# HuttleyLab/DiverseSeq

Measured on NVIDIA B200. Metric: prep_nmost_throughput, higher is better.
Workload: dtype u8 bases -> u32 counts -> f64 frequencies/entropy/JSD

## Files before the change

diverseseq_b200/csrc/select.cu:

```cuda
#include <limits.h>
#include <stddef.h>
#include <stdlib.h>
#include <string.h>

#include <algorithm>
#include <limits>

#include <cooperative_groups.h>

#include "comm.cuh"
#include "common.cuh"
#include "entropy.cuh"
#include "fused.cuh"

namespace cg = cooperative_groups;

namespace dvs {

constexpr unsigned kNone = 0xFFFFFFFFu;

struct SelScal {
    double E;
    double total_jsd;
    double mean, stdv, cov;
// ... 523 lines not shown
                cudaOccupancyMaxActiveBlocksPerMultiprocessor(&per_sm2, k_sel_persist_sm_full, kFastThreads,
                                                              sizeof(SmShared)) == cudaSuccess &&
                per_sm2 > 0;
        (void)cudaGetLastError();
    }
    const unsigned sm_grid = std::min(std::min<unsigned>((unsigned)ctx->sm_count, kSmMaxGrid), grid_cap);
    const int slim_threads = 128 * (trail_shape() + 1);
    const auto k_slim = slim_threads == 384 ? SlimKernel<384>::fn : (slim_threads == 256 ? SlimKernel<256>::fn : SlimKernel<128>::fn);
    bool slim_ok = false;
    if (trail && sm_ok) {
        slim_ok = cudaFuncSetAttribute(k_slim, cudaFuncAttributeMaxDynamicSharedMemorySize,
                                       (int)sizeof(SmSharedSlim)) == cudaSuccess &&
                  cudaFuncSetAttribute(k_slim, cudaFuncAttributePreferredSharedMemoryCarveout,
                                       (int)cudaSharedmemCarveoutMaxShared) == cudaSuccess;
        (void)cudaGetLastError();
    }
    DevBuf<SlicePart> d_slparts;
    DevBuf<unsigned> d_slticks;
    DevBuf<SmPart> d_spart, d_upart, d_dpart;
    if (sm_ok) {
        DVS_TRY(d_spart.alloc(2 * kSmMaxGrid));
        DVS_TRY(d_upart.alloc(kSmMaxN + 1));
        DVS_TRY(d_dpart.alloc(3));
    }
    const char* gb_env = getenv("DVS_SELECT_GROW_BATCH");
    const bool use_grow_batch = use_fast && grow_mode && !(gb_env && gb_env[0] == '0');
    const unsigned kGrowWindowMax = 64 * world;
    SelState fresh;
    DevBuf<FastSum> d_gparts;
    DevBuf<double> d_gmd, d_gmb;
    DevBuf<SelScal> d_gscratch;
    DevBuf<unsigned> d_ginteresting;
    bool fresh_valid = false;
    unsigned grow_window = 16;
    if (use_grow_batch && n != max_size) {
        DVS_TRY(fresh.alloc(dim, cap));
        DVS_TRY(d_gparts.alloc((size_t)kGrowWindowMax * (cap + 3)));
        DVS_TRY(d_gmd.alloc((size_t)kGrowWindowMax * cap));
        DVS_TRY(d_gmb.alloc((size_t)kGrowWindowMax * cap));
        DVS_TRY(d_gscratch.alloc(kGrowWindowMax));
        DVS_TRY(d_ginteresting.alloc(1));
    }
    unsigned fresh_n = 0;
    const SelState* fresh_of = nullptr;
    int fresh_which = -1;
    bool single_candidate = false;
    unsigned filter_streak = 0, filter_bypass = 0;
    while (cursor < num) {
        if (use_grow_batch && n != max_size && !single_candidate && filter_bypass > 0) {
            --filter_bypass;
            single_candidate = true;
            continue;
        }
        if (use_grow_batch && n != max_size && !single_candidate) {
            if (!fresh_valid || fresh_n != n || fresh_of != cur || fresh_which != cur->which) {
                k_sel_sum<<<sel.vec_grid(), 256, 0, st>>>(f->freqs.p, f->entropy.p, dim, cur->members(), n, -1, fresh.S(),
                                                          fresh.members(), fresh.sc.p);
                DVS_LAUNCHED(ctx);
                fresh_valid = true;
                fresh_n = n;
                fresh_of = cur;
                fresh_which = cur->which;
            }
            const unsigned W = std::min(grow_window, num - cursor);
            DVS_CUDA_TRY(cudaMemsetAsync(d_ginteresting.p, 0xFF, sizeof(unsigned), st));
            const unsigned gc0 = (rank + world - cursor % world) % world;
            const unsigned Wloc = W > gc0 ? (W - gc0 + world - 1) / world : 0;
            if (Wloc) {
                k_grow_eval<<<dim3(n + 3, Wloc), kFastThreads, 0, st>>>(f->freqs.p, dim, cur->S(), cur->members(), cur->sc.p,
                                                                        fresh.S(), f->valid.p, is_member.p, d_order.p,
                                                                        cursor, d_gparts.p, gc0, world);
                DVS_LAUNCHED(ctx);
                k_grow_decide<<<Wloc, kFastThreads, 0, st>>>(f->entropy.p, dim, cur->members(), cur->sc.p, fresh.sc.p,
                                                             f->valid.p, is_member.p, d_order.p, cursor, d_gparts.p, d_gmd.p,
                                                             d_gmb.p, cap, d_gscratch.p, d_ginteresting.p,
                                                             mode == DVS_MODE_MAX_COV ? 1 : 0, gc0, world);
                DVS_LAUNCHED(ctx);
            }
            if (world > 1) DVS_TRY(comm_min_u32(ctx, comm, d_ginteresting.p, d_ginteresting.p));
            unsigned* h_fi = reinterpret_cast<unsigned*>(reinterpret_cast<char*>(ctx->pinned) + sizeof(SelScal));
            DVS_CUDA_TRY(cudaMemcpyAsync(h_fi, d_ginteresting.p, sizeof(unsigned), cudaMemcpyDeviceToHost, st));
            DVS_CUDA_TRY(cudaStreamSynchronize(st));
            const unsigned fi = *h_fi;
            if (fi == kNone) {
                cursor += W;
                grow_window = std::min(grow_window * 2u, kGrowWindowMax);
                continue;
            }
            grow_window = std::max(4u, std::min(kGrowWindowMax, 2u * (fi - cursor + 1u)));
            if (fi == cursor) {
                if (++filter_streak >= 2) filter_bypass = 1u << std::min(filter_streak - 2u, 3u);
            } else {
                filter_streak = 0;
            }
            cursor = fi;
            single_candidate = true;
            continue;
        }
        if (trail && trail_limit < num && !use_persist) {
            DVS_CUDA_TRY(cudaStreamWaitEvent(st, trail->count_done, 0));
            trail_limit = num;
        }
        if (use_persist && (!grow_mode || n == max_size)) {
            const bool use_sm = sm_ok && n <= kSmMaxN;
            const bool dedicated = trail_shape() == 3;
            const bool trailing = trail && trail_limit < num && use_sm && world == 1 &&
                                  (dedicated || (slim_ok && n <= kSmSlimMaxN));
            if (trail && trail_limit < num && !trailing) {
                DVS_CUDA_TRY(cudaStreamWaitEvent(st, trail->count_done, 0));
                trail_limit = num;
            }
            const unsigned grid = (trailing && dedicated) ? std::min(sm_grid, trail_sms(ctx->sm_count))
                                                           : (use_sm ? sm_grid : persist_grid);
            k_sel_set_dev<<<1, 1, 0, st>>>(cur->sc.p, cursor, std::min(window, grid * world), grid * world, num, accepts,
                                           (unsigned)cur->which);
            if (comm) {
                shard.tag_base = (unsigned)((++comm->sel_tag_base) << 20);
                DVS_TRY(comm_host_rendezvous(ctx, comm));
            }
            DVS_LAUNCHED(ctx);
            const double* a_F = f->freqs.p;
            const double* a_H = f->entropy.p;
            uint64_t a_dim = dim;
            double *a_S0 = cur->Sbuf[0].p, *a_S1 = cur->Sbuf[1].p;
            unsigned *a_M0 = cur->membuf[0].p, *a_M1 = cur->membuf[1].p;
            uint8_t* a_mem = is_member.p;
            double *a_md = cur->mdelta.p, *a_mb = cur->mbound.p;
            SelScal* a_sc = cur->sc.p;
            const uint8_t* a_valid = f->valid.p;
            const unsigned* a_order = d_order.p;
            unsigned a_rounds = world > 1 ? 0xFFFF0u : 0x7fffffffu;
            unsigned long long* a_trace = nullptr;
            DevBuf<unsigned long long> d_trace;
            const char* tr_env = getenv("DVS_SELECT_TRACE");
            const char* tra_env = getenv("DVS_SELECT_TRACE_ALL");
            int a_trace_all = (use_sm && tra_env && tra_env[0]) ? 1 : 0;
            const size_t trace_len = a_trace_all ? (size_t)256 * kSmTraceSlots * kSmMaxGrid : 2048;
            if (a_trace_all) tr_env = nullptr;
            if ((tr_env && tr_env[0]) || a_trace_all) {
                DVS_TRY(d_trace.alloc(trace_len));
                DVS_CUDA_TRY(cudaMemsetAsync(d_trace.p, 0, trace_len * sizeof(unsigned long long), st));
                a_trace = d_trace.p;
            }
            if (use_sm) {
                unsigned a_dim32 = (unsigned)dim;
                double* a_S = cur->S();
                unsigned* a_M = cur->members();
                SmPart *a_sp = d_spart.p, *a_up = d_upart.p, *a_dp = d_dpart.p;
                DVS_CUDA_TRY(cudaMemsetAsync(d_dpart.p, 0, 3 * sizeof(SmPart), st));
                DVS_CUDA_TRY(cudaMemsetAsync(d_spart.p, 0, 2 * kSmMaxGrid * sizeof(SmPart), st));
                DVS_CUDA_TRY(cudaMemsetAsync(d_upart.p, 0, (kSmMaxN + 1) * sizeof(SmPart), st));
                const unsigned* a_ready = trailing ? trail->d_ready : nullptr;
                unsigned a_limit0 = trail_limit;
                void* args[] = {&a_F, &a_H, &a_dim32, &a_S, &a_M, &a_mem, &a_md, &a_mb, &a_sc, &a_valid, &a_order,
                                &a_sp, &a_up, &a_dp, &a_trace, &a_trace_all, &shard, &a_ready, &a_limit0};
                if (trailing && dedicated) {
                    if (!ctx->stream_hi) {
                        int lo_p = 0, hi_p = 0;
                        DVS_CUDA_TRY(cudaDeviceGetStreamPriorityRange(&lo_p, &hi_p));
                        DVS_CUDA_TRY(cudaStreamCreateWithPriority(&ctx->stream_hi, cudaStreamNonBlocking, hi_p));
                        DVS_CUDA_TRY(cudaEventCreateWithFlags(&ctx->ev_hi_in, cudaEventDisableTiming));
                        DVS_CUDA_TRY(cudaEventCreateWithFlags(&ctx->ev_hi_out, cudaEventDisableTiming));
                    }
                    DVS_CUDA_TRY(cudaEventRecord(ctx->ev_hi_in, st));
                    DVS_CUDA_TRY(cudaStreamWaitEvent(ctx->stream_hi, ctx->ev_hi_in, 0));
                    k_sel_persist_sm_full<<<grid, kFastThreads, sizeof(SmShared), ctx->stream_hi>>>(
                        a_F, a_H, a_dim32, a_S, a_M, a_mem, a_md, a_mb, a_sc, a_valid, a_order, a_sp, a_up, a_dp, a_trace,
                        a_trace_all, shard, a_ready, a_limit0);
                    DVS_CUDA_TRY(cudaGetLastError());
                    DVS_CUDA_TRY(cudaEventRecord(ctx->ev_hi_out, ctx->stream_hi));
                    DVS_CUDA_TRY(cudaStreamWaitEvent(st, ctx->ev_hi_out, 0));
                } else if (trailing) {
                    k_wait_resident<<<1, 1, 0, st>>>(trail->d_resident, std::min<unsigned>(grid, (unsigned)ctx->sm_count),
                                                     trail->d_ready, num);
                    DVS_LAUNCHED(ctx);
                }
                if (trailing && dedicated) {
                } else if (trailing)
                    k_slim<<<grid, slim_threads, sizeof(SmSharedSlim), st>>>(
                        a_F, a_H, a_dim32, a_S, a_M, a_mem, a_md, a_mb, a_sc, a_valid, a_order, a_sp, a_up, a_dp, a_trace,
                        a_trace_all, shard, a_ready, a_limit0);
                else
                    DVS_CUDA_TRY(cudaLaunchCooperativeKernel((void*)k_sel_persist_sm_full, dim3(grid), dim3(kFastThreads),
                                                             args, sizeof(SmShared), st));
            } else {
                const char* sl_env = getenv("DVS_SELECT_SLICES");
                unsigned a_slice_mode = sl_env ? (unsigned)atoi(sl_env) : 1u;
                if (!d_slparts.p && a_slice_mode) {
                    const size_t slots = std::max<size_t>(grid, (size_t)cap + 1);
                    DVS_TRY(d_slparts.alloc(slots * kMaxSlices));
                    DVS_TRY(d_slticks.alloc(slots));
                    DVS_CUDA_TRY(cudaMemsetAsync(d_slticks.p, 0, slots * sizeof(unsigned), st));
                }
                SlicePart* a_parts = d_slparts.p;
                unsigned* a_ticks = d_slticks.p;
                void* args[] = {&a_F, &a_H, &a_dim, &a_S0, &a_S1, &a_M0, &a_M1, &a_mem, &a_md, &a_mb, &a_sc, &a_valid,
                                &a_order, &a_rounds, &a_trace, &shard, &a_parts, &a_ticks, &a_slice_mode};
                DVS_CUDA_TRY(cudaLaunchCooperativeKernel((void*)k_sel_persist, dim3(grid), dim3(kFastThreads), args, 0, st));
            }
            ctx->launches++;
            DVS_TRY(sel.read(*cur));
            if (a_trace && a_trace_all) {
                std::vector<unsigned long long> tr(trace_len);
                DVS_CUDA_TRY(cudaMemcpy(tr.data(), a_trace, trace_len * sizeof(unsigned long long), cudaMemcpyDeviceToHost));
                if (FILE* fp = fopen(tra_env, "wb")) {
                    fwrite(tr.data(), sizeof(unsigned long long), trace_len, fp);
                    fclose(fp);
                }
            } else if (a_trace) {
                std::vector<unsigned long long> tr(2048);
                DVS_CUDA_TRY(cudaMemcpy(tr.data(), a_trace, 2048 * sizeof(unsigned long long), cudaMemcpyDeviceToHost));
                if (FILE* fp = fopen(tr_env, "a")) {
                    const int slots = use_sm ? kSmTraceSlots : 4, used = use_sm ? 7 : 4;
                    fprintf(fp, use_sm ? "# round scan_ns gather_ns decide_ns update_ns gather2_ns finalize_ns next_ns (CTA 0)\n"
                                       : "# round scan_ns wait1_ns update_ns wait2_ns (CTA 0; wait = grid barrier incl. the slowest CTA)\n");
                    for (int r = 0; (r + 1) * slots < 2048 && tr[slots * (r + 1)]; ++r) {
                        fprintf(fp, "%d", r);
                        for (int q = 0; q + 1 < used; ++q) fprintf(fp, " %llu", tr[slots * r + q + 1] - tr[slots * r + q]);
                        fprintf(fp, " %llu\n", tr[slots * (r + 1)] - tr[slots * r + used - 1]);
                    }
                    fclose(fp);
                }
            }
            const SelScal hd = *sel.h_sc;
            if (hd.panic) return panic_error(hd);
            if (trailing) {
                ctx->last_trail_accepts += hd.accepts - accepts;
                ++ctx->last_trail_launches;
                std::vector<unsigned> smid(grid);
                DVS_CUDA_TRY(cudaMemcpyAsync(smid.data(), trail->d_ready + kTrailSmidOff, grid * sizeof(unsigned),
                                             cudaMemcpyDeviceToHost, st));
                DVS_CUDA_TRY(cudaStreamSynchronize(st));
                std::sort(smid.begin(), smid.end());
                const unsigned distinct = (unsigned)(std::unique(smid.begin(), smid.end()) - smid.begin());
                ctx->last_trail_sms = std::min(ctx->last_trail_sms, distinct);
            }
            cursor = hd.cursor;
            window = hd.window;
            accepts = hd.accepts;
            cur->which = (int)hd.which;
            if (trailing) trail_limit = std::max(trail_limit, std::min(hd.limit, num));
            if (!hd.halt) continue;
            DVS_TRY(sel.reset_scan(*cur));
            if (cursor >= num) break;
        } else if (use_dev && world == 1 && (!grow_mode || n == max_size)) {
            k_sel_set_dev<<<1, 1, 0, st>>>(cur->sc.p, cursor, std::min(window, window_max_dev), window_max_dev, num,
                                           accepts, (unsigned)cur->which);
            DVS_LAUNCHED(ctx);
            for (int r = 0; r < kRoundsPerBatch; ++r) {
                k_sel_scan_dev<<<window_max_dev, kFastThreads, 0, st>>>(
                    f->freqs.p, f->entropy.p, dim, cur->Sbuf[0].p, cur->Sbuf[1].p, cur->membuf[0].p, cur->membuf[1].p,
                    cur->sc.p, f->valid.p, is_member.p, d_order.p);
                DVS_LAUNCHED(ctx);
                k_sel_round_dev<<<n + 1, kFastThreads, 0, st>>>(
                    f->freqs.p, f->entropy.p, dim, cur->Sbuf[0].p, cur->Sbuf[1].p, cur->membuf[0].p, cur->membuf[1].p,
                    is_member.p, cur->mdelta.p, cur->mbound.p, cur->sc.p, d_order.p);
                DVS_LAUNCHED(ctx);
            }
            DVS_TRY(sel.read(*cur));
            const SelScal hd = *sel.h_sc;
            if (hd.panic) return panic_error(hd);
            cursor = hd.cursor;
            window = hd.window;
            accepts = hd.accepts;
            cur->which = (int)hd.which;
            if (!hd.halt) continue;
            DVS_TRY(sel.reset_scan(*cur));
            if (cursor >= num) break;
        }
        if (cursor >= trail_limit) {
            DVS_CUDA_TRY(cudaStreamWaitEvent(st, trail->count_done, 0));
            trail_limit = num;
        }
        const unsigned count = single_candidate ? 1u : std::min(window, trail_limit - cursor);
        single_candidate = false;
        SelScal h;
        unsigned pos = kNone;
        if (use_fast) {
            DVS_TRY(sel.scan_fast(*cur, is_member.p, d_order.p, cursor, count));
            DVS_TRY(sel.read(*cur));
            h = *sel.h_sc;
            if (h.panic) return panic_error(h);
            if (h.state_unsure) {
                DVS_TRY(sel.update(*cur, n));
                ++exact_evals;
                continue;
            }
            if (h.first_unsure < h.first_true) {
                const unsigned pu = h.first_unsure;
                if (!h.exact) DVS_TRY(sel.update(*cur, n));
                DVS_TRY(sel.scan(*cur, f, is_member.p, d_order.p, pu, 1, nullptr));
                DVS_TRY(sel.read(*cur));
                h = *sel.h_sc;
                ++exact_evals;
                if (h.panic) return panic_error(h);
                if (h.first_panic == pu) {
                    set_error("cannot calculate entropy as frequency vector total !=1.0 (candidate at position %u)", pu);
                    return DVS_ERR_VALUE;
                }
                if (h.first_true != pu) {
                    DVS_TRY(sel.reset_scan(*cur));
                    cursor = pu + 1;
                    continue;
                }
                pos = pu;
            } else if (h.first_true != kNone) {
                pos = h.first_true;
            }
        } else {
            DVS_TRY(sel.scan(*cur, f, is_member.p, d_order.p, cursor, count, nullptr));
            DVS_TRY(sel.read(*cur));
            h = *sel.h_sc;
            if (h.panic) return panic_error(h);
            if (h.first_panic != kNone && h.first_panic <= h.first_true) {
                set_error("cannot calculate entropy as frequency vector total !=1.0 (candidate at position %u)",
                          h.first_panic);
                return DVS_ERR_VALUE;
            }
            pos = h.first_true;
        }
        if (pos == kNone) {
            cursor += count;
            window = std::min(window * 2, window_max);
            continue;
        }
        const unsigned row = order[pos];
        window = std::max(64u, std::min(window_max, 2 * (pos - cursor + 1)));
        cursor = pos + 1;
        if (!grow_mode || n == max_size) {
            DVS_TRY(use_fast ? sel.replace_fast(*cur, n, row, is_member.p) : sel.replace(*cur, n, row, is_member.p));
            ++accepts;
            continue;
        }
        const bool use_cov = (mode == DVS_MODE_MAX_COV);
// ... 279 lines not shown
```

diverseseq_b200/csrc/select_fast.cuh:

```cuda
#pragma once

constexpr int kFastThreads = 512;

struct FastSum {
    double e, t, a;
    int bad;
};

template <class Elem>
__device__ FastSum block_entropy_span(uint64_t lo, uint64_t dim, Elem elem) {
    __shared__ double s_part[3][kFastThreads / 32];
    __shared__ int s_bad[kFastThreads / 32];
    double e0 = 0.0, e1 = 0.0, t0 = 0.0, t1 = 0.0, a0 = 0.0, a1 = 0.0;
    int bad = 0;
    constexpr int kBatch = 8;
    for (uint64_t base = lo; base < dim; base += (uint64_t)kBatch * kFastThreads) {
        double x[kBatch];
#pragma unroll
        for (int q = 0; q < kBatch; ++q) {
            const uint64_t i = base + threadIdx.x + (uint64_t)q * kFastThreads;
            x[q] = i < dim ? elem(i) : 0.0;
        }
#pragma unroll
        for (int q = 0; q < kBatch; q += 2) {
            const double x0 = x[q], x1 = x[q + 1];
            if (!(x0 == 0.0)) {
                bad |= !(x0 > 0.0);
                const double tm = __dmul_rn(-x0, log2(x0));
                e0 += tm; a0 += fabs(tm); t0 += x0;
            }
            if (!(x1 == 0.0)) {
                bad |= !(x1 > 0.0);
                const double tm = __dmul_rn(-x1, log2(x1));
                e1 += tm; a1 += fabs(tm); t1 += x1;
            }
        }
    }
    double e = e0 + e1, t = t0 + t1, a = a0 + a1;
    for (int o = 16; o; o >>= 1) {
        e += __shfl_xor_sync(0xffffffffu, e, o);
        t += __shfl_xor_sync(0xffffffffu, t, o);
        a += __shfl_xor_sync(0xffffffffu, a, o);
        bad |= __shfl_xor_sync(0xffffffffu, bad, o);
    }
    const int w = threadIdx.x >> 5;
    if ((threadIdx.x & 31) == 0) {
        s_part[0][w] = e; s_part[1][w] = t; s_part[2][w] = a; s_bad[w] = bad;
    }
    __syncthreads();
    FastSum r{0.0, 0.0, 0.0, 0};
    for (int q = 0; q < kFastThreads / 32; ++q) {
        r.e += s_part[0][q]; r.t += s_part[1][q]; r.a += s_part[2][q]; r.bad |= s_bad[q];
    }
    __syncthreads();
    return r;
}
template <class Elem>
__device__ __forceinline__ FastSum block_entropy_fast(uint64_t dim, Elem elem) {
    return block_entropy_span(0, dim, elem);
}

__device__ __forceinline__ bool fast_term_ok(double m) {
    return (uint32_t)__double2hiint(m) - 0x07b00000u < 0x3feea4afu - 0x07b00000u;
}

template <bool CLAMP, int BATCH, int NT = kFastThreads, class Num>
__device__ FastSum block_entropy_ilp(unsigned lo, unsigned hi, Num num, const FastDiv dv,
                                     const double2* __restrict__ ltab) {
    __shared__ double s_part[3][NT / 32];
    __shared__ int s_bad[NT / 32];
    double e0 = 0.0, e1 = 0.0, t0 = 0.0, t1 = 0.0, a0 = 0.0, a1 = 0.0;
    bool bad = false;
    for (unsigned base = lo; base < hi; base += BATCH * NT) {
        double x[BATCH], l[BATCH];
#pragma unroll
        for (int q = 0; q < BATCH; ++q) {
            const unsigned i = base + threadIdx.x + (unsigned)q * NT;
            x[q] = i < hi ? num(i) : 0.0;
        }
#pragma unroll
        for (int q = 0; q < BATCH; ++q) {
            double m = div_exact(x[q], dv);
            if (CLAMP) m = (m <= kEps) ? 0.0 : m;
            x[q] = m;
        }
#pragma unroll
        for (int q = 0; q < BATCH; ++q) {
            int ignored = 0;
            l[q] = dvs_log2_main(x[q], ltab, ignored);
        }
#pragma unroll
        for (int q = 0; q < BATCH; ++q) {
            const bool ok = fast_term_ok(x[q]);
            bad |= !ok && !(x[q] == 0.0);
            const double tm = ok ? __dmul_rn(-x[q], l[q]) : 0.0;
            if (q & 1) {
                e1 += tm; a1 += fabs(tm); t1 += x[q];
            } else {
                e0 += tm; a0 += fabs(tm); t0 += x[q];
            }
        }
    }
    double e = e0 + e1, t = t0 + t1, a = a0 + a1;
    int badi = bad ? 1 : 0;
    for (int o = 16; o; o >>= 1) {
        e += __shfl_xor_sync(0xffffffffu, e, o);
        t += __shfl_xor_sync(0xffffffffu, t, o);
        a += __shfl_xor_sync(0xffffffffu, a, o);
        badi |= __shfl_xor_sync(0xffffffffu, badi, o);
    }
    const int w = threadIdx.x >> 5;
    if ((threadIdx.x & 31) == 0) {
        s_part[0][w] = e; s_part[1][w] = t; s_part[2][w] = a; s_bad[w] = badi;
    }
    __syncthreads();
    FastSum r{0.0, 0.0, 0.0, 0};
    for (int q = 0; q < NT / 32; ++q) {
        r.e += s_part[0][q]; r.t += s_part[1][q]; r.a += s_part[2][q]; r.bad |= s_bad[q];
    }
    __syncthreads();
    return r;
}

template <bool CLAMP, class Num>
__device__ FastSum block_entropy_div(uint64_t dim, Num num, double divisor) {
    if (dim > (1ull << 30) || !(divisor >= 1.0 && divisor <= 4096.0)) {
        return block_entropy_fast(dim, [&](uint64_t i) {
            const double m = __ddiv_rn(num(i), divisor);
            return (CLAMP && m <= kEps) ? 0.0 : m;
        });
    }
    __shared__ double2 s_ltab_div[64];
    dvs_log2_stage_table(s_ltab_div);
    __syncthreads();
    return block_entropy_ilp<CLAMP, 8>(0u, (unsigned)dim, num, make_fast_div(divisor), s_ltab_div);
}

__device__ __forceinline__ double fast_slack(uint64_t dim, double depth = 0.0) {
    return (double)(dim / kFastThreads) + 12.0 + depth;
}
__device__ __forceinline__ double fast_bound(uint64_t dim, double a, double extra, double depth = 0.0) {
    return ((double)dim + fast_slack(dim, depth) + 16.0) * 1.2e-16 * (a + fabs(extra) + 1.0);
}
__device__ __forceinline__ bool fast_total_ok(uint64_t dim, double t, double depth = 0.0) {
    const double lim = ((double)dim + 1.0 - fast_slack(dim, depth) - 2.0) * 1.1102230246251565e-16;
    return lim > 0.0 && fabs(t - 1.0) <= lim;
}

template <bool GLOBAL = true>
__device__ __forceinline__ unsigned finalize_fast_block(double* mdelta, const double* mbound, unsigned n, double total,
                                                        double total_bound, unsigned* low_out) {
    auto ld = [](const double* p) { return GLOBAL ? __ldcg(p) : *p; };
    __shared__ double s_mn[kFastThreads / 32], s_mb[kFastThreads / 32];
    __shared__ unsigned s_ix[kFastThreads / 32];
    __shared__ double s_best, s_bestb;
    __shared__ unsigned s_besti;
    double mn = 1e300, mb = 0.0;
    unsigned ix = kNone;
    for (unsigned t = threadIdx.x; t < n; t += blockDim.x) {
        const double d = total - ld(&mdelta[t]);
        mdelta[t] = d;
        if (d < mn || (d == mn && t < ix)) {
            mn = d;
            mb = ld(&mbound[t]);
            ix = t;
        }
    }
    for (int o = 16; o; o >>= 1) {
        const double omn = __shfl_xor_sync(0xffffffffu, mn, o), omb = __shfl_xor_sync(0xffffffffu, mb, o);
        const unsigned oix = __shfl_xor_sync(0xffffffffu, ix, o);
        if (omn < mn || (omn == mn && oix < ix)) {
            mn = omn; mb = omb; ix = oix;
        }
    }
    if ((threadIdx.x & 31) == 0) {
        s_mn[threadIdx.x >> 5] = mn; s_mb[threadIdx.x >> 5] = mb; s_ix[threadIdx.x >> 5] = ix;
    }
    __syncthreads();
    if (threadIdx.x == 0) {
        for (unsigned w = 1; w < blockDim.x / 32; ++w)
            if (s_mn[w] < mn || (s_mn[w] == mn && s_ix[w] < ix)) {
                mn = s_mn[w]; mb = s_mb[w]; ix = s_ix[w];
            }
        s_best = mn; s_bestb = mb; s_besti = (ix == kNone) ? 0u : ix;
    }
    __syncthreads();
    mn = s_best; mb = s_bestb;
    const unsigned low = s_besti;
    int unsure = 0;
    for (unsigned t = threadIdx.x; t < n; t += blockDim.x)
        if (t != low && !(mn + mb + 2.0 * kEps < mdelta[t] - ld(&mbound[t]))) unsure = 1;
    if (!(mn + mb + total_bound < 1e6)) unsure = 1;
    unsure = __syncthreads_or(unsure);
    *low_out = low;
    return (unsigned)unsure;
}

__device__ __forceinline__ double block_sum_fast(double v) {
    __shared__ double s_red[kFastThreads / 32];
    __shared__ double s_out;
    for (int o = 16; o; o >>= 1) v += __shfl_xor_sync(0xffffffffu, v, o);
    if ((threadIdx.x & 31) == 0) s_red[threadIdx.x >> 5] = v;
    __syncthreads();
    if (threadIdx.x == 0) {
        double t = 0.0;
        for (unsigned w = 0; w < blockDim.x / 32; ++w) t += s_red[w];
        s_out = t;
    }
    __syncthreads();
    const double r = s_out;
    __syncthreads();
    return r;
}
__device__ __forceinline__ double block_max_fast(double v) {
    __shared__ double s_red[kFastThreads / 32];
    __shared__ double s_out;
    for (int o = 16; o; o >>= 1) v = fmax(v, __shfl_xor_sync(0xffffffffu, v, o));
    if ((threadIdx.x & 31) == 0) s_red[threadIdx.x >> 5] = v;
    __syncthreads();
    if (threadIdx.x == 0) {
        double t = s_red[0];
        for (unsigned w = 1; w < blockDim.x / 32; ++w) t = fmax(t, s_red[w]);
        s_out = t;
    }
    __syncthreads();
    const double r = s_out;
    __syncthreads();
    return r;
}

__device__ __forceinline__ void stats_fast_block(const double* mdelta, const double* mbound, unsigned n,
                                                 double total_bound, SelScal* sc) {
    double sd = 0.0, bmx = 0.0, amx = 0.0;
    for (unsigned t = threadIdx.x; t < n; t += blockDim.x) {
        const double d = mdelta[t];
        sd += d;
        bmx = fmax(bmx, __ldcg(&mbound[t]));
        amx = fmax(amx, fabs(d));
    }
    const double nd = (double)n;
    const double mean = block_sum_fast(sd) / nd;
    bmx = block_max_fast(bmx);
    amx = block_max_fast(amx);
    double ss = 0.0;
    for (unsigned t = threadIdx.x; t < n; t += blockDim.x) {
        const double d = mdelta[t] - mean;
        ss += d * d;
    }
    const double sdev = sqrt(block_sum_fast(ss) / (nd - 1.0));
    if (threadIdx.x == 0) {
        const double u = 1.2e-16, scale = amx + fabs(mean);
        const double b_mean = bmx + total_bound + (nd + 8.0) * u * scale;
        const double b_std = 1.5 * (bmx + 4.0 * u * scale) + (nd + 8.0) * u * sdev;
        const double cov = sdev / mean;
        double b_cov = 1e300;
        if (fabs(mean) > 2.0 * b_mean) b_cov = (b_std + fabs(cov) * b_mean) / (fabs(mean) - b_mean) + 8.0 * u * fabs(cov);
        sc->mean = mean;
        sc->stdv = sdev;
        sc->cov = cov;
        sc->std_bound = b_std;
        sc->cov_bound = b_cov;
    }
}

struct ScanScal {
    double E, total_jsd, total_bound;
    unsigned n, low_row;
};

__device__ __forceinline__ void scan_fast_body(const double* __restrict__ F, const double* __restrict__ H, uint64_t dim,
                                               const double* __restrict__ S, SelScal* sc, const ScanScal& q,
                                               const uint8_t* __restrict__ valid,
                                               const uint8_t* __restrict__ is_member,
                                               const unsigned* __restrict__ order, unsigned pos) {
    const unsigned row = order[pos];
    if (!valid[row] || __ldcg(is_member + row)) return;
    const double nd = (double)q.n;
    const double* fl = F + (size_t)q.low_row * dim;
    const double* fc = F + (size_t)row * dim;
    FastSum h = block_entropy_div<false>(
        dim, [&](uint64_t i) { return __dadd_rn(__dsub_rn(__ldcg(S + i), fl[i]), fc[i]); }, nd);
    if (threadIdx.x == 0) {
        const double mean_entropy = __ddiv_rn(__dadd_rn(__dsub_rn(q.E, H[q.low_row]), H[row]), nd);
        const double d = h.e - mean_entropy;
        const double b = fast_bound(dim, h.a, mean_entropy);
        const double thr = q.total_jsd + kEps, tb = q.total_bound + 4.0 * kEps;
        if (h.bad || !fast_total_ok(dim, h.t) || !(d == d)) {
            atomicMin(&sc->first_unsure, pos);
        } else if (d - b > thr + tb) {
            atomicMin(&sc->first_true, pos);
        } else if (!(d + b < thr - tb)) {
            atomicMin(&sc->first_unsure, pos);
// ... 471 lines not shown
```

diverseseq_b200/csrc/select_sm.cuh:

```cuda
#pragma once

constexpr unsigned kSmMaxDim = 4096, kSmMaxN = 1024, kSmMaxGrid = 256, kSmChunk = 4 * kFastThreads;
constexpr double kSmDepth = 4.0;

struct __align__(16) SmPart {
    unsigned long long w[4];
};

template <unsigned MAXN, unsigned CHUNK>
struct SmSharedT {
    double S[kSmMaxDim];
    double mH[2][MAXN + 1];
    double md[MAXN + 1];
    double mb[MAXN + 1];
    unsigned members[2][MAXN + 1];
    double cH[CHUNK];
    unsigned crow[CHUNK];
    unsigned char cvalid[CHUNK];
    double pe[kSmMaxGrid], pt[kSmMaxGrid], pa[kSmMaxGrid];
    unsigned char pbad[kSmMaxGrid], wskip[kSmMaxGrid];
    unsigned ft, fu, unsure, xft, xfu, dead, limit;
    double2 ltab[64];
};
using SmShared = SmSharedT<kSmMaxN, kSmChunk>;
constexpr unsigned kSmSlimMaxN = 256, kSmSlimChunk = 1280;
using SmSharedSlim = SmSharedT<kSmSlimMaxN, kSmSlimChunk>;

__device__ __forceinline__ void sm_st128(void* p, unsigned long long lo, unsigned long long hi) {
    asm volatile("{ .reg .b128 v; mov.b128 v, {%1, %2}; st.relaxed.gpu.global.b128 [%0], v; }" ::"l"(p), "l"(lo), "l"(hi)
                 : "memory");
}
__device__ __forceinline__ void sm_ld128(const void* p, unsigned long long& lo, unsigned long long& hi) {
    asm volatile("{ .reg .b128 v; ld.relaxed.gpu.global.b128 v, [%2]; mov.b128 {%0, %1}, v; }"
                 : "=l"(lo), "=l"(hi)
                 : "l"(p)
                 : "memory");
}
__device__ __forceinline__ void sm_publish(SmPart* slot, const FastSum& h, unsigned tag) {
    sm_st128(&slot->w[0], (unsigned long long)__double_as_longlong(h.e), ((unsigned long long)(h.bad ? 1u : 0u) << 32) | tag);
    sm_st128(&slot->w[2], (unsigned long long)__double_as_longlong(h.t),
             ((unsigned long long)__float_as_uint(__double2float_ru(h.a)) << 32) | tag);
}
__device__ __forceinline__ FastSum sm_gather(const SmPart* slot, unsigned tag) {
    unsigned long long w0, w1, w2, w3;
    do sm_ld128(&slot->w[0], w0, w1); while ((unsigned)w1 != tag);
    do sm_ld128(&slot->w[2], w2, w3); while ((unsigned)w3 != tag);
    return FastSum{__longlong_as_double((long long)w0), __longlong_as_double((long long)w2),
                   (double)__uint_as_float((unsigned)(w3 >> 32)), (int)(w1 >> 32)};
}

template <int NT>
__device__ __forceinline__ unsigned sm_finalize(double* md, const double* mb_, unsigned n, double total,
                                                double total_bound, unsigned* low_out) {
    __shared__ double s_mn[NT / 32], s_mb[NT / 32];
    __shared__ unsigned s_ix[NT / 32];
    double mn = 1e300, mb = 0.0;
    unsigned ix = kNone;
    for (unsigned t = threadIdx.x; t < n; t += blockDim.x) {
        const double d = total - md[t];
        md[t] = d;
        if (d < mn || (d == mn && t < ix)) {
            mn = d; mb = mb_[t]; ix = t;
        }
    }
    for (int o = 16; o; o >>= 1) {
        const double omn = __shfl_xor_sync(0xffffffffu, mn, o), omb = __shfl_xor_sync(0xffffffffu, mb, o);
        const unsigned oix = __shfl_xor_sync(0xffffffffu, ix, o);
        if (omn < mn || (omn == mn && oix < ix)) {
            mn = omn; mb = omb; ix = oix;
        }
    }
    if ((threadIdx.x & 31) == 0) {
        s_mn[threadIdx.x >> 5] = mn; s_mb[threadIdx.x >> 5] = mb; s_ix[threadIdx.x >> 5] = ix;
    }
    __syncthreads();
    mn = s_mn[0]; mb = s_mb[0]; ix = s_ix[0];
#pragma unroll
    for (unsigned w = 1; w < NT / 32; ++w) {
        const double wmn = s_mn[w];
        const unsigned wix = s_ix[w];
        if (wmn < mn || (wmn == mn && wix < ix)) {
            mn = wmn; mb = s_mb[w]; ix = wix;
        }
    }
    const unsigned low = (ix == kNone) ? 0u : ix;
    int unsure = 0;
    for (unsigned t = threadIdx.x; t < n; t += blockDim.x)
        if (t != low && !(mn + mb + 2.0 * kEps < md[t] - mb_[t])) unsure = 1;
    if (!(mn + mb + total_bound < 1e6)) unsure = 1;
    unsure = __syncthreads_or(unsure);
    *low_out = low;
    return (unsigned)unsure;
}

constexpr int kSmTraceSlots = 8;
constexpr unsigned kTrailSmidOff = 64;

template <int NT, int MINB, unsigned MAXN, unsigned CHUNK>
__global__ void __launch_bounds__(NT, MINB)
k_sel_persist_sm_t(const double* __restrict__ F, const double* __restrict__ H, unsigned dim, double* S_glob,
                 unsigned* M_glob, uint8_t* is_member, double* mdelta_g, double* mbound_g, SelScal* sc,
                 const uint8_t* __restrict__ valid, const unsigned* __restrict__ order, SmPart* spart, SmPart* upart,
                 SmPart* dpart, unsigned long long* trace, int trace_all, const ShardArgs sh,
                 const unsigned* ready_pos, unsigned limit0) {
    extern __shared__ __align__(16) unsigned char sm_raw[];
    SmSharedT<MAXN, CHUNK>& sm = *reinterpret_cast<SmSharedT<MAXN, CHUNK>*>(sm_raw);
    const unsigned tid = threadIdx.x, b = blockIdx.x, G = gridDim.x;
    if (ready_pos && tid == 0) {
        unsigned smid;
        asm volatile("mov.u32 %0, %%smid;" : "=r"(smid));
        const_cast<unsigned*>(ready_pos)[kTrailSmidOff + b] = smid;
    }
    unsigned tr_round = 0;
    auto stamp = [&](int slot) {
        if (trace && tid == 0 && tr_round < 256 && (b == 0 || trace_all)) {
            unsigned long long t;
            asm volatile("mov.u64 %0, %%globaltimer;" : "=l"(t));
            if (trace_all)
                trace[((size_t)tr_round * kSmTraceSlots + slot) * kSmMaxGrid + b] = t;
            else
                trace[tr_round * kSmTraceSlots + slot] = t;
        }
    };

    const unsigned n = sc->n, num = sc->num;
    const double nd = (double)n, div = __dsub_rn(nd, 1.0);
    const FastDiv div_n = make_fast_div(nd), div_n1 = make_fast_div(div);
    double E = sc->E, total_jsd = sc->total_jsd, total_bound = sc->total_bound;
    unsigned lowest = sc->lowest, cursor = sc->cursor, window = sc->window, accepts = sc->accepts;
    unsigned state_unsure = sc->state_unsure, halt = state_unsure ? 1u : 0u, mw = 0;
    bool touched = false;
    dvs_log2_stage_table(sm.ltab);
    for (unsigned i = tid; i < dim; i += NT) sm.S[i] = S_glob[i];
    for (unsigned j = tid; j < n; j += NT) {
        const unsigned r = M_glob[j];
        sm.members[0][j] = r;
        sm.mH[0][j] = H[r];
    }
    __syncthreads();
    const unsigned world = (unsigned)sh.world, rank = (unsigned)sh.rank, Gw = G * world;
    const unsigned wmin = max(1u, Gw / 4u);
    if (tid == 0) sm.dead = 0;
    const double kb0 = ((double)dim + fast_slack(dim) + 16.0) * 1.2e-16;
    const double kb4 = ((double)dim + fast_slack(dim, kSmDepth) + 16.0) * 1.2e-16;
    const double lim0 = ((double)dim + 1.0 - fast_slack(dim) - 2.0) * 1.1102230246251565e-16;
    const double lim4 = ((double)dim + 1.0 - fast_slack(dim, kSmDepth) - 2.0) * 1.1102230246251565e-16;
    auto total_ok = [](double t, double lim) { return lim > 0.0 && fabs(t - 1.0) <= lim; };
    unsigned xs = 0, xu = 0;
    unsigned cbase = 0, cend = 0;
    unsigned limit = ready_pos ? min(limit0, num) : num;

    while (!halt && cursor < num) {
        stamp(0);
        if (xs >= 0xFFFF0u) {
            halt = 1;
            break;
        }
        if (ready_pos && limit >= num) break;
        window = max(1u, min(window, min(Gw, CHUNK)));
        const unsigned P = (dim >= 2048u && window * 4u <= Gw) ? 4u : ((dim >= 2048u && window * 2u <= Gw) ? 2u : 1u);
        const unsigned count = min(window, limit - cursor);
        const unsigned woff = (rank + world - cursor % world) % world;
        const unsigned nloc = count > woff ? (count - woff + world - 1u) / world : 0u;
        if (cursor < cbase || cursor + count > cend) {
            __syncthreads();
            cbase = cursor;
            cend = min(limit, cbase + CHUNK);
            for (unsigned q = tid; cbase + q < cend; q += NT) {
                const unsigned row = order[cbase + q];
                sm.crow[q] = row;
                sm.cvalid[q] = __ldcg(valid + row);
                sm.cH[q] = __ldcg(H + row);
            }
            for (unsigned r = (rank + world - cbase % world) % world + world * b; r < cend - cbase; r += world * G) {
                const double* fr = F + (size_t)order[cbase + r] * dim;
                for (unsigned l = tid * 16u; l < dim; l += NT * 16u)
                    asm volatile("prefetch.global.L2 [%0];" ::"l"(fr + l));
            }
            __syncthreads();
        }
        const unsigned coff = cursor - cbase;
        if (tid == 0) {
            sm.ft = kNone;
            sm.fu = kNone;
        }
        for (unsigned q = tid; q < nloc; q += NT) sm.wskip[q] = sm.cvalid[coff + woff + world * q] ? 0 : 1;
        ++xs;
        SmPart* const sbuf = spart + (xs & 1u) * kSmMaxGrid;
        const unsigned c = b / P, p = b % P;
        const unsigned cw = woff + world * c;
        const double* fl = F + (size_t)sm.members[mw][lowest] * dim;
        if (c < nloc && sm.cvalid[coff + cw]) {
            const double* fc = F + (size_t)sm.crow[coff + cw] * dim;
            const unsigned lo = (unsigned)(((uint64_t)dim * p) / P), hi = (unsigned)(((uint64_t)dim * (p + 1)) / P);
            auto num = [&](unsigned i) { return __dadd_rn(__dsub_rn(sm.S[i], fl[i]), fc[i]); };
            const FastSum h = P == 4u   ? block_entropy_ilp<false, 2, NT>(lo, hi, num, div_n, sm.ltab)
                              : P == 2u ? block_entropy_ilp<false, 4, NT>(lo, hi, num, div_n, sm.ltab)
                                        : block_entropy_ilp<false, 8, NT>(lo, hi, num, div_n, sm.ltab);
            if (tid == 0) sm_publish(sbuf + b, h, xs);
        } else if (tid == 0) {
            sm_publish(sbuf + b, FastSum{0.0, 0.0, 0.0, 0}, xs);
        }
        stamp(1);
        SmPart* const dslot = dpart + (xs & 1u);
        if (b == 0) {
            __syncthreads();
            for (unsigned j = tid; j < n; j += NT) {
                const unsigned r = sm.members[mw][j];
                for (unsigned cc = 0; cc < nloc; ++cc)
                    if (sm.crow[coff + woff + world * cc] == r) sm.wskip[cc] = 1;
            }
            __syncthreads();
            for (unsigned q = tid; q < G; q += NT) {
                const FastSum g = sm_gather(sbuf + q, xs);
                if (q < nloc * P && !sm.wskip[q / P]) {
                    sm.pe[q] = g.e; sm.pt[q] = g.t; sm.pa[q] = g.a; sm.pbad[q] = (unsigned char)g.bad;
                }
            }
            __syncthreads();
            stamp(2);
            for (unsigned lc = tid; lc < nloc; lc += NT) {
                if (sm.wskip[lc]) continue;
                FastSum h{sm.pe[lc * P], sm.pt[lc * P], sm.pa[lc * P], sm.pbad[lc * P]};
                for (unsigned q = 1; q < P; ++q) {
                    h.e += sm.pe[lc * P + q]; h.t += sm.pt[lc * P + q]; h.a += sm.pa[lc * P + q];
                    h.bad |= sm.pbad[lc * P + q];
                }
                const unsigned pos = cursor + woff + world * lc;
                const double mean_entropy =
                    div_exact(__dadd_rn(__dsub_rn(E, sm.mH[mw][lowest]), sm.cH[pos - cbase]), div_n);
                const double d = h.e - mean_entropy;
                const double bd = (P > 1u ? kb4 : kb0) * (h.a + fabs(mean_entropy) + 1.0);
                const double thr = total_jsd + kEps, tb = total_bound + 4.0 * kEps;
                if (h.bad || !total_ok(h.t, P > 1u ? lim4 : lim0) || !(d == d)) {
                    atomicMin(&sm.fu, pos);
                } else if (d - bd > thr + tb) {
                    atomicMin(&sm.ft, pos);
                } else if (!(d + bd < thr - tb)) {
                    atomicMin(&sm.fu, pos);
                }
            }
            __syncthreads();
            if (world > 1u) {
                const unsigned lft = sm.ft, lfu = sm.fu;
                __syncthreads();
                shard_exchange_min(sh, xs, lft, lfu, &sm.ft, &sm.fu, &sm.dead);
                __syncthreads();
                if (sm.dead) {
                    if (tid == 0) {
                        sm.ft = kNone;
                        sm.fu = 0u;
                        sc->panic = 2u;
                    }
                    __syncthreads();
                }
            }
            if (tid == 0) {
                unsigned nl = limit;
                if (ready_pos) nl = max(limit, min(num, *reinterpret_cast<const volatile unsigned*>(ready_pos)));
                sm.limit = nl;
                sm_st128(&dslot->w[0], ((unsigned long long)sm.fu << 32) | sm.ft, ((unsigned long long)nl << 32) | xs);
            }
            __syncthreads();
        } else {
            if (tid == 0) {
                unsigned long long w0, w1;
                do sm_ld128(&dslot->w[0], w0, w1); while ((unsigned)w1 != xs);
                sm.ft = (unsigned)w0;
                sm.fu = (unsigned)(w0 >> 32);
                sm.limit = (unsigned)(w1 >> 32);
            }
            stamp(2);
            __syncthreads();
        }
        const unsigned ft = sm.ft, fu = sm.fu;
        const unsigned next_limit = sm.limit;
        __syncthreads();
        stamp(3);
        if (fu < ft) {
            halt = 1;
            break;
        }
        if (ft == kNone) {
            cursor += count;
            if (count) window = min(window * 2u, Gw);
            limit = next_limit;
            stamp(4); stamp(5); stamp(6);
            ++tr_round;
            continue;
        }
        const unsigned cand = sm.crow[ft - cbase];
        const double Hc = sm.cH[ft - cbase];
        const double E_new = __dadd_rn(__dsub_rn(E, sm.mH[mw][lowest]), Hc);
        const double* fc = F + (size_t)cand * dim;
        auto member_after = [&](unsigned j) {
            return j < lowest ? sm.members[mw][j] : (j + 1 < n ? sm.members[mw][j + 1] : cand);
        };
        auto s_new = [&](unsigned i) {
            double s = __dsub_rn(sm.S[i], fl[i]);
            if (s <= kEps) s = 0.0;
            return __dadd_rn(s, fc[i]);
        };
        ++xu;
        bool have_S = false;
        for (unsigned j = b; j <= n; j += G) {
            FastSum h;
            if (j == n) {
                h = block_entropy_ilp<false, 8, NT>(0u, dim, [&](unsigned i) {
                    const double s = have_S ? sm.S[i] : s_new(i);
                    if (!have_S) sm.S[i] = s;
                    return s;
                }, div_n, sm.ltab);
            } else {
                const double* f = F + (size_t)member_after(j) * dim;
                h = block_entropy_ilp<true, 8, NT>(0u, dim, [&](unsigned i) {
                    const double s = have_S ? sm.S[i] : s_new(i);
                    if (!have_S) sm.S[i] = s;
                    return __dsub_rn(s, f[i]);
                }, div_n1, sm.ltab);
            }
            if (tid == 0) sm_publish(upart + j, h, xu);
            have_S = true;
        }
        if (!have_S)
            for (unsigned i = tid; i < dim; i += NT) sm.S[i] = s_new(i);
        stamp(4);
        for (unsigned t = tid; t < n; t += NT) {
            sm.members[mw ^ 1][t] = member_after(t);
            sm.mH[mw ^ 1][t] = t < lowest ? sm.mH[mw][t] : (t + 1 < n ? sm.mH[mw][t + 1] : Hc);
        }
        if (tid == 0) sm.unsure = 0;
        __syncthreads();
        mw ^= 1;
        E = E_new;
        unsigned lo2 = 0, unsure = 0;
        SmPart* const fslot = dpart + 2;
        if (b == 0) {
            int uns = 0;
            for (unsigned t = tid; t <= n; t += NT) {
                const FastSum g = sm_gather(upart + t, xu);
                if (t == n) {
                    sm.pe[0] = g.e; sm.pa[0] = g.a;
                } else {
                    const double mean_entropy = div_exact(__dsub_rn(E, sm.mH[mw][t]), div_n1);
                    sm.md[t] = g.e - mean_entropy;
                    sm.mb[t] = kb0 * (g.a + fabs(mean_entropy) + 1.0);
                }
                if (g.bad || !total_ok(g.t, lim0)) uns = 1;
            }
            if (uns) sm.unsure = 1;
            __syncthreads();
            stamp(5);
            const double me = div_exact(E, div_n);
            total_jsd = sm.pe[0] - me;
            total_bound = kb0 * (sm.pa[0] + fabs(me) + 1.0);
            unsure = sm_finalize<NT>(sm.md, sm.mb, n, total_jsd, total_bound, &lo2);
            unsure |= sm.unsure;
            if (tid == 0) {
                sm_st128(&fslot->w[0], (unsigned long long)__double_as_longlong(total_jsd), ((unsigned long long)lo2 << 32) | xu);
                sm_st128(&fslot->w[2], (unsigned long long)__double_as_longlong(total_bound),
                         ((unsigned long long)unsure << 32) | xu);
            }
        } else {
            if (tid == 0) {
                unsigned long long w0, w1, w2, w3;
                do sm_ld128(&fslot->w[0], w0, w1); while ((unsigned)w1 != xu);
                do sm_ld128(&fslot->w[2], w2, w3); while ((unsigned)w3 != xu);
                sm.pe[0] = __longlong_as_double((long long)w0);
                sm.pa[0] = __longlong_as_double((long long)w2);
                sm.ft = (unsigned)(w1 >> 32);
                sm.unsure = (unsigned)(w3 >> 32);
            }
            __syncthreads();
            stamp(5);
            total_jsd = sm.pe[0];
            total_bound = sm.pa[0];
            lo2 = sm.ft;
            unsure = sm.unsure;
            __syncthreads();
        }
        lowest = lo2;
        touched = true;
        limit = next_limit;
        window = max(wmin, min(Gw, 2u * (ft - cursor + 1u)));
        cursor = ft + 1u;
        ++accepts;
        stamp(6);
        ++tr_round;
        if (unsure) {
            state_unsure = 1;
            halt = 1;
            break;
        }
    }
    stamp(0);

    if (b == 0) {
        __syncthreads();
        if (touched) {
            for (unsigned i = tid; i < dim; i += NT) S_glob[i] = sm.S[i];
            for (unsigned j = tid; j < n; j += NT) is_member[M_glob[j]] = 0;
            __syncthreads();
            for (unsigned j = tid; j < n; j += NT) {
                const unsigned r = sm.members[mw][j];
                M_glob[j] = r;
                is_member[r] = 1;
                mdelta_g[j] = sm.md[j];
                mbound_g[j] = sm.mb[j];
            }
        }
        if (tid == 0) {
            if (touched) {
                sc->E = E;
                sc->total_jsd = total_jsd;
                sc->total_bound = total_bound;
                sc->lowest = lowest;
                sc->exact = 0;
            }
            sc->state_unsure = state_unsure;
            sc->ticket = 0;
            sc->first_true = kNone;
            sc->first_panic = kNone;
            sc->first_unsure = kNone;
            sc->cursor = cursor;
            sc->window = window;
            sc->accepts = accepts;
            sc->halt = halt;
            sc->limit = limit;
        }
    }
}
```

Baseline: 3407.

## Split persistent block into warp groups evaluating multiple update slots concurrently

In the shared-memory persistent selection kernel, each 512-thread block is now split into up to 8 warp groups, selected by DVS_SELECT_SLOT_GROUPS with a default of 8. Each group evaluates a different member slot's entropy concurrently instead of the whole block walking the slots one after another, and groups synchronise through named barriers. The candidate-updated S vector is written to a new shared buffer Sn and copied back afterwards, which adds shared memory and an extra copy. The error bounds are widened to match the smaller per-group thread count, which may make more results fall into the unsure path.

```diff
diff --git a/diverseseq_b200/csrc/select.cu b/diverseseq_b200/csrc/select.cu
--- a/diverseseq_b200/csrc/select.cu
+++ b/diverseseq_b200/csrc/select.cu
@@ -699,8 +699,10 @@
                 DVS_CUDA_TRY(cudaMemsetAsync(d_upart.p, 0, (kSmMaxN + 1) * sizeof(SmPart), st));
                 const unsigned* a_ready = trailing ? trail->d_ready : nullptr;
                 unsigned a_limit0 = trail_limit;
+                const char* ug_env = getenv("DVS_SELECT_SLOT_GROUPS");
+                unsigned a_groups = ug_env && atoi(ug_env) > 0 ? (unsigned)atoi(ug_env) : 8u;
                 void* args[] = {&a_F, &a_H, &a_dim32, &a_S, &a_M, &a_mem, &a_md, &a_mb, &a_sc, &a_valid, &a_order,
-                                &a_sp, &a_up, &a_dp, &a_trace, &a_trace_all, &shard, &a_ready, &a_limit0};
+                                &a_sp, &a_up, &a_dp, &a_trace, &a_trace_all, &shard, &a_ready, &a_limit0, &a_groups};
                 if (trailing && dedicated) {
                     if (!ctx->stream_hi) {
                         int lo_p = 0, hi_p = 0;
@@ -713,7 +715,7 @@
                     DVS_CUDA_TRY(cudaStreamWaitEvent(ctx->stream_hi, ctx->ev_hi_in, 0));
                     k_sel_persist_sm_full<<<grid, kFastThreads, sizeof(SmShared), ctx->stream_hi>>>(
                         a_F, a_H, a_dim32, a_S, a_M, a_mem, a_md, a_mb, a_sc, a_valid, a_order, a_sp, a_up, a_dp, a_trace,
-                        a_trace_all, shard, a_ready, a_limit0);
+                        a_trace_all, shard, a_ready, a_limit0, a_groups);
                     DVS_CUDA_TRY(cudaGetLastError());
                     DVS_CUDA_TRY(cudaEventRecord(ctx->ev_hi_out, ctx->stream_hi));
                     DVS_CUDA_TRY(cudaStreamWaitEvent(st, ctx->ev_hi_out, 0));
@@ -726,7 +728,7 @@
                 } else if (trailing)
                     k_slim<<<grid, slim_threads, sizeof(SmSharedSlim), st>>>(
                         a_F, a_H, a_dim32, a_S, a_M, a_mem, a_md, a_mb, a_sc, a_valid, a_order, a_sp, a_up, a_dp, a_trace,
-                        a_trace_all, shard, a_ready, a_limit0);
+                        a_trace_all, shard, a_ready, a_limit0, a_groups);
                 else
                     DVS_CUDA_TRY(cudaLaunchCooperativeKernel((void*)k_sel_persist_sm_full, dim3(grid), dim3(kFastThreads),
                                                              args, sizeof(SmShared), st));
diff --git a/diverseseq_b200/csrc/select_fast.cuh b/diverseseq_b200/csrc/select_fast.cuh
--- a/diverseseq_b200/csrc/select_fast.cuh
+++ b/diverseseq_b200/csrc/select_fast.cuh
@@ -64,18 +64,26 @@
     return (uint32_t)__double2hiint(m) - 0x07b00000u < 0x3feea4afu - 0x07b00000u;
 }
 
-template <bool CLAMP, int BATCH, int NT = kFastThreads, class Num>
+template <bool CLAMP, int BATCH, int NT = kFastThreads, int GT = NT, class Num>
 __device__ FastSum block_entropy_ilp(unsigned lo, unsigned hi, Num num, const FastDiv dv,
                                      const double2* __restrict__ ltab) {
+    static_assert(NT % GT == 0 && GT % 32 == 0, "groups are whole warps");
     __shared__ double s_part[3][NT / 32];
     __shared__ int s_bad[NT / 32];
+    const unsigned gtid = threadIdx.x % GT, w0 = (threadIdx.x - gtid) / 32;
+    auto group_sync = [&]() {
+        if (GT == NT)
+            __syncthreads();
+        else
+            asm volatile("bar.sync %0, %1;" ::"r"(1u + threadIdx.x / GT), "r"(GT) : "memory");
+    };
     double e0 = 0.0, e1 = 0.0, t0 = 0.0, t1 = 0.0, a0 = 0.0, a1 = 0.0;
     bool bad = false;
-    for (unsigned base = lo; base < hi; base += BATCH * NT) {
+    for (unsigned base = lo; base < hi; base += BATCH * GT) {
         double x[BATCH], l[BATCH];
 #pragma unroll
         for (int q = 0; q < BATCH; ++q) {
-            const unsigned i = base + threadIdx.x + (unsigned)q * NT;
+            const unsigned i = base + gtid + (unsigned)q * GT;
             x[q] = i < hi ? num(i) : 0.0;
         }
 #pragma unroll
@@ -113,12 +121,12 @@
     if ((threadIdx.x & 31) == 0) {
         s_part[0][w] = e; s_part[1][w] = t; s_part[2][w] = a; s_bad[w] = badi;
     }
-    __syncthreads();
+    group_sync();
     FastSum r{0.0, 0.0, 0.0, 0};
-    for (int q = 0; q < NT / 32; ++q) {
+    for (unsigned q = w0; q < w0 + GT / 32; ++q) {
         r.e += s_part[0][q]; r.t += s_part[1][q]; r.a += s_part[2][q]; r.bad |= s_bad[q];
     }
-    __syncthreads();
+    group_sync();
     return r;
 }
 
@@ -136,8 +144,9 @@
     return block_entropy_ilp<CLAMP, 8>(0u, (unsigned)dim, num, make_fast_div(divisor), s_ltab_div);
 }
 
-__device__ __forceinline__ double fast_slack(uint64_t dim, double depth = 0.0) {
-    return (double)(dim / kFastThreads) + 12.0 + depth;
+__host__ __device__ __forceinline__ double fast_slack(uint64_t dim, double depth = 0.0,
+                                                      unsigned threads = kFastThreads) {
+    return (double)(dim / threads) + 12.0 + depth;
 }
 __device__ __forceinline__ double fast_bound(uint64_t dim, double a, double extra, double depth = 0.0) {
     return ((double)dim + fast_slack(dim, depth) + 16.0) * 1.2e-16 * (a + fabs(extra) + 1.0);
diff --git a/diverseseq_b200/csrc/select_sm.cuh b/diverseseq_b200/csrc/select_sm.cuh
--- a/diverseseq_b200/csrc/select_sm.cuh
+++ b/diverseseq_b200/csrc/select_sm.cuh
@@ -7,9 +7,10 @@
     unsigned long long w[4];
 };
 
-template <unsigned MAXN, unsigned CHUNK>
+template <unsigned MAXN, unsigned CHUNK, unsigned SNDIM = kSmMaxDim>
 struct SmSharedT {
     double S[kSmMaxDim];
+    double Sn[SNDIM];
     double mH[2][MAXN + 1];
     double md[MAXN + 1];
     double mb[MAXN + 1];
@@ -24,7 +25,7 @@
 };
 using SmShared = SmSharedT<kSmMaxN, kSmChunk>;
 constexpr unsigned kSmSlimMaxN = 256, kSmSlimChunk = 1280;
-using SmSharedSlim = SmSharedT<kSmSlimMaxN, kSmSlimChunk>;
+using SmSharedSlim = SmSharedT<kSmSlimMaxN, kSmSlimChunk, 1>;
 
 __device__ __forceinline__ void sm_st128(void* p, unsigned long long lo, unsigned long long hi) {
     asm volatile("{ .reg .b128 v; mov.b128 v, {%1, %2}; st.relaxed.gpu.global.b128 [%0], v; }" ::"l"(p), "l"(lo), "l"(hi)
@@ -93,6 +94,16 @@
     return (unsigned)unsure;
 }
 
+template <int V>
+struct SmGroupThreads {
+    static constexpr int value = V;
+};
+__host__ __device__ __forceinline__ unsigned sm_update_groups(unsigned slots, unsigned max_groups) {
+    unsigned g = 1;
+    while (g < slots && g < max_groups && g < 8u) g *= 2u;
+    return g;
+}
+
 constexpr int kSmTraceSlots = 8;
 constexpr unsigned kTrailSmidOff = 64;
 
@@ -102,9 +113,10 @@
                  unsigned* M_glob, uint8_t* is_member, double* mdelta_g, double* mbound_g, SelScal* sc,
                  const uint8_t* __restrict__ valid, const unsigned* __restrict__ order, SmPart* spart, SmPart* upart,
                  SmPart* dpart, unsigned long long* trace, int trace_all, const ShardArgs sh,
-                 const unsigned* ready_pos, unsigned limit0) {
+                 const unsigned* ready_pos, unsigned limit0, unsigned max_groups) {
     extern __shared__ __align__(16) unsigned char sm_raw[];
-    SmSharedT<MAXN, CHUNK>& sm = *reinterpret_cast<SmSharedT<MAXN, CHUNK>*>(sm_raw);
+    using Shared = SmSharedT<MAXN, CHUNK, NT == kFastThreads ? kSmMaxDim : 1u>;
+    Shared& sm = *reinterpret_cast<Shared*>(sm_raw);
     const unsigned tid = threadIdx.x, b = blockIdx.x, G = gridDim.x;
     if (ready_pos && tid == 0) {
         unsigned smid;
@@ -145,6 +157,9 @@
     const double kb4 = ((double)dim + fast_slack(dim, kSmDepth) + 16.0) * 1.2e-16;
     const double lim0 = ((double)dim + 1.0 - fast_slack(dim) - 2.0) * 1.1102230246251565e-16;
     const double lim4 = ((double)dim + 1.0 - fast_slack(dim, kSmDepth) - 2.0) * 1.1102230246251565e-16;
+    const unsigned ugroups = NT == kFastThreads ? sm_update_groups((n + G) / G, max_groups) : 1u;
+    const double kbu = ((double)dim + fast_slack(dim, 0.0, NT / ugroups) + 16.0) * 1.2e-16;
+    const double limu = ((double)dim + 1.0 - fast_slack(dim, 0.0, NT / ugroups) - 2.0) * 1.1102230246251565e-16;
     auto total_ok = [](double t, double lim) { return lim > 0.0 && fabs(t - 1.0) <= lim; };
     unsigned xs = 0, xu = 0;
     unsigned cbase = 0, cend = 0;
@@ -302,28 +317,53 @@
             return __dadd_rn(s, fc[i]);
         };
         ++xu;
-        bool have_S = false;
-        for (unsigned j = b; j <= n; j += G) {
-            FastSum h;
-            if (j == n) {
-                h = block_entropy_ilp<false, 8, NT>(0u, dim, [&](unsigned i) {
-                    const double s = have_S ? sm.S[i] : s_new(i);
-                    if (!have_S) sm.S[i] = s;
-                    return s;
-                }, div_n, sm.ltab);
-            } else {
-                const double* f = F + (size_t)member_after(j) * dim;
-                h = block_entropy_ilp<true, 8, NT>(0u, dim, [&](unsigned i) {
-                    const double s = have_S ? sm.S[i] : s_new(i);
-                    if (!have_S) sm.S[i] = s;
-                    return __dsub_rn(s, f[i]);
-                }, div_n1, sm.ltab);
-            }
-            if (tid == 0) sm_publish(upart + j, h, xu);
-            have_S = true;
-        }
-        if (!have_S)
-            for (unsigned i = tid; i < dim; i += NT) sm.S[i] = s_new(i);
+        auto update_slots = [&](auto gt) {
+            constexpr int GT = decltype(gt)::value;
+            constexpr bool kInPlace = GT == NT;
+            double* const Sd = kInPlace ? sm.S : sm.Sn;
+            const unsigned q = tid / GT;
+            auto eval = [&](unsigned j, bool first) {
+                const bool store = first && q == 0;
+                FastSum h;
+                if (j == n) {
+                    h = block_entropy_ilp<false, 8, NT, GT>(0u, dim, [&](unsigned i) {
+                        if (!first) return Sd[i];
+                        const double s = s_new(i);
+                        if (store) Sd[i] = s;
+                        return s;
+                    }, div_n, sm.ltab);
+                } else {
+                    const double* f = F + (size_t)member_after(j) * dim;
+                    h = block_entropy_ilp<true, 8, NT, GT>(0u, dim, [&](unsigned i) {
+                        double s;
+                        if (first) {
+                            s = s_new(i);
+                            if (store) Sd[i] = s;
+                        } else {
+                            s = Sd[i];
+                        }
+                        return __dsub_rn(s, f[i]);
+                    }, div_n1, sm.ltab);
+                }
+                if (tid % GT == 0) sm_publish(upart + j, h, xu);
+            };
+            unsigned j = b + G * q;
+            if (j <= n) eval(j, true);
+            else if (q == 0)
+                for (unsigned i = tid; i < dim; i += GT) Sd[i] = s_new(i);
+            if (b + G * (NT / GT) <= n || !kInPlace) __syncthreads();
+            for (j += G * (NT / GT); j <= n; j += G * (NT / GT)) eval(j, false);
+            if (!kInPlace)
+                for (unsigned i = tid; i < dim; i += NT) sm.S[i] = sm.Sn[i];
+        };
+        if constexpr (NT == kFastThreads) {
+            if (ugroups == 8u) update_slots(SmGroupThreads<NT / 8>{});
+            else if (ugroups == 4u) update_slots(SmGroupThreads<NT / 4>{});
+            else if (ugroups == 2u) update_slots(SmGroupThreads<NT / 2>{});
+            else update_slots(SmGroupThreads<NT>{});
+        } else {
+            update_slots(SmGroupThreads<NT>{});
+        }
         stamp(4);
         for (unsigned t = tid; t < n; t += NT) {
             sm.members[mw ^ 1][t] = member_after(t);
@@ -344,16 +384,16 @@
                 } else {
                     const double mean_entropy = div_exact(__dsub_rn(E, sm.mH[mw][t]), div_n1);
                     sm.md[t] = g.e - mean_entropy;
-                    sm.mb[t] = kb0 * (g.a + fabs(mean_entropy) + 1.0);
-                }
-                if (g.bad || !total_ok(g.t, lim0)) uns = 1;
+                    sm.mb[t] = kbu * (g.a + fabs(mean_entropy) + 1.0);
+                }
+                if (g.bad || !total_ok(g.t, limu)) uns = 1;
             }
             if (uns) sm.unsure = 1;
             __syncthreads();
             stamp(5);
             const double me = div_exact(E, div_n);
             total_jsd = sm.pe[0] - me;
-            total_bound = kb0 * (sm.pa[0] + fabs(me) + 1.0);
+            total_bound = kbu * (sm.pa[0] + fabs(me) + 1.0);
             unsure = sm_finalize<NT>(sm.md, sm.mb, n, total_jsd, total_bound, &lo2);
             unsure |= sm.unsure;
             if (tid == 0) {
```

New measurement: 3047 (median of 6 runs). 0.894x the previous value.
